# michel-aractingi/soloRL

Hardware: AMD Instinct MI355X
Metric: env-steps/s (whole node) Solo12 walk, 4096 envs/GPU (higher is better)
Workload: dtype f32

## Files before the change

### solorl_amd/csrc/dynamics.hpp

```cpp
#pragma once
#include <utility>

#include "../../include/solorl.h"
#include "../../include/solorl_model_data.h"
#include "spatial.hpp"

namespace solo {

constexpr int MAX_CONTACTS = 8;
constexpr int MAX_LIMITS = 4;
constexpr int LIM_SLOT_ROWS = 2;
constexpr int MAX_ROWS = LIM_SLOT_ROWS + 3 * MAX_CONTACTS;
SD int extra_limits(int nlt) { return nlt > LIM_SLOT_ROWS ? nlt - LIM_SLOT_ROWS : 0; }
SD int contact_cap(int nlt) { return MAX_CONTACTS - extra_limits(nlt); }
constexpr int ROW_CORE = 20;
constexpr int NPRIM = 24;
constexpr double LIMIT_WINDOW = 0.0;
constexpr double DISC_EPS2 = 1e-12;
constexpr double DISC_RIM = 0.1;

#if defined(SOLO_WAVE_TIMING) && !defined(SOLO_HOST_SHIM)
constexpr int SOLO_WT_WAVES = 65536, SOLO_WT_FIELDS = 30;
__device__ unsigned long long solo_wave_times[SOLO_WT_WAVES][SOLO_WT_FIELDS];
__shared__ unsigned long long solo_pt_acc[12];
#define SOLO_PT_DECL() long long pt_last_ = 0
#define SOLO_PT_BEGIN() do { __builtin_amdgcn_s_waitcnt(0); pt_last_ = clock64(); } while (0)
#define SOLO_PT(i) do { __builtin_amdgcn_s_waitcnt(0); if (threadIdx.x == 0) { const long long n_ = clock64(); solo_pt_acc[i] += (unsigned long long)(n_ - pt_last_); } pt_last_ = clock64(); } while (0)
#else
#define SOLO_PT_DECL() do {} while (0)
#define SOLO_PT_BEGIN() do {} while (0)
#define SOLO_PT(i) do {} while (0)
#endif

template <int N, typename F, int... I>
SD void static_for_impl(F&& f, std::integer_sequence<int, I...>) { (f(std::integral_constant<int, I>{}), ...); }
template <int N, typename F> SD void static_for(F&& f) { static_for_impl<N>(f, std::make_integer_sequence<int, N>{}); }

template <int ROBOT> struct Robot;
template <> struct Robot<0> {
  static constexpr int NJ = 2, NQ = 8, NL = 13;
  static constexpr bool SHOULDER = false;
  static constexpr const solorl_model_data& MD = SOLORL_MODEL_SOLO8;
};
template <> struct Robot<1> {
  static constexpr int NJ = 3, NQ = 12, NL = 17;
  static constexpr bool SHOULDER = true;
  static constexpr const solorl_model_data& MD = SOLORL_MODEL_SOLO12;
};

constexpr bool base_points_are_sign_patterns(const solorl_model_data& md) {
  const solorl_prim_data& a = md.prims[0]; const solorl_prim_data& b = md.prims[8];
  for (int p = 0; p < 12; p++) {
    const solorl_prim_data& q = md.prims[p];
    const bool plate = p >= 8;
    const double sx = ((plate ? (p - 8) >> 1 : p >> 2) & 1) ? -1.0 : 1.0, sy = ((plate ? (p - 8) : p >> 1) & 1) ? -1.0 : 1.0;
    const double cx = (plate ? b.center[0] : a.center[0]) * sx, cy = (plate ? b.center[1] : a.center[1]) * sy;
    const double cz = plate ? b.center[2] : ((p & 1) ? -a.center[2] : a.center[2]);
    if (q.link != 0 || q.axis != -1 || q.center[0] != cx || q.center[1] != cy || q.center[2] != cz || q.margin != a.margin || q.friction != a.friction) return false;
  }
  return true;
}

template <typename T> struct PhysParams {
  T dt, gravity, erp, slop, warm, damping, vmax, qlim, inv_dt;
  int iterations;
  T tm_hw, tm_mu;
  T resid_thr;
  T cerp;
  T cmargin;
  int mode;
  enum { M_PIPE = 1, M_URDF = 2, M_CONE = 4, M_TREADMILL = 8 };
  SD bool pgs_pipe() const { return mode & M_PIPE; }
  SD bool urdf_inertia() const { return mode & M_URDF; }
  SD bool cone() const { return mode & M_CONE; }
  SD bool tm_on() const { return mode & M_TREADMILL; }
  void set_mode(bool pipe, bool urdf, bool cone_, bool treadmill) {
    mode = (pipe ? M_PIPE : 0) | (urdf ? M_URDF : 0) | (cone_ ? M_CONE : 0) | (treadmill ? M_TREADMILL : 0);
  }
};
template <typename T> PhysParams<T> make_phys(const solorl_config& c) {
  PhysParams<T> p;
  p.dt = (T)c.sim_dt; p.gravity = (T)c.gravity; p.erp = (T)c.erp; p.slop = (T)c.linear_slop; p.warm = (T)c.warmstart;
  p.damping = (T)c.damping; p.vmax = (T)c.max_velocity; p.qlim = (T)c.joint_limit; p.inv_dt = (T)(1.0 / c.sim_dt);
  p.iterations = c.solver_iterations;
  p.tm_hw = (T)c.treadmill_half_width; p.tm_mu = (T)c.treadmill_friction;
  p.resid_thr = c.solver_residual_threshold > 0 ? (T)std::sqrt(c.solver_residual_threshold) : T(-1);
  p.cerp = (T)c.contact_erp; p.cmargin = (T)c.collision_margin;
  p.set_mode(true, c.use_urdf_inertia != 0, c.friction_model == SOLORL_FRICTION_CONE, c.use_treadmill != 0);
  return p;
}
SD int strip_feet_bits(int smask) {
  return (((smask >> 13) & 1) << 24) | (((smask >> 15) & 1) << 25) | (((smask >> 17) & 1) << 26) | (((smask >> 19) & 1) << 27);
}

template <typename T, int NQ> struct PhysState {
  V3<T> pos; T qx, qy, qz, qw; V3<T> v, w;
  T q[NQ], qd[NQ];
};

template <typename T> struct JointF { SV<T> S, U, c; T Dinv, u; };

#ifndef SOLO_HOST_SHIM
extern __shared__ __attribute__((aligned(16))) unsigned char solo_smem_sym[];
#if defined(SOLO_WAVE_TIMING)
constexpr unsigned SOLO_LDS_BASE = 96;
#else
constexpr unsigned SOLO_LDS_BASE = 0;
#endif
typedef __attribute__((address_space(3))) unsigned char solo_lds_byte;
#define solo_smem (((unsigned char*)reinterpret_cast<solo_lds_byte*>(SOLO_LDS_BASE + 4096u)) - 4096)
#endif
#ifdef SOLO_HOST_SHIM
template <typename T> constexpr int default_lanes() { return 1; }
#else
template <typename T> constexpr int default_lanes() { return sizeof(T) == 4 ? 64 : 32; }
#endif
template <typename T, int LN = default_lanes<T>()> struct RowLds {
  static constexpr int PER = 16 / sizeof(T);
  static constexpr int NCH = ROW_CORE / PER;
  static constexpr int LANES = LN;
  using Chunk = typename std::conditional<sizeof(T) == 4, float4, double2>::type;
  enum { A_MU = 0, A_LAM = 1, A_YOFF = 2, A_META = 3 };
  int lanes, lane;
#ifdef SOLO_HOST_SHIM
  unsigned char* base;
  SD unsigned char* smem() const { return base; }
#else
  SD unsigned char* smem() const { return solo_smem; }
#endif
  SD Chunk* core() const { return reinterpret_cast<Chunk*>(smem()) + lane; }
  SD T* aux() const { return reinterpret_cast<T*>(smem() + (size_t)MAX_ROWS * LANES * ROW_CORE * sizeof(T)) + lane; }
  SD T* y() const { return reinterpret_cast<T*>(smem() + (size_t)MAX_ROWS * LANES * (ROW_CORE + 4) * sizeof(T)) + lane; }
  SD T* hdr() const { return y() + 12 * LANES; }
  SD T& A(int r, int f) const { return aux()[(r * 4 + f) * LANES]; }

  SD void store_core(int r, const T (&v)[ROW_CORE]) const {
    Chunk* p = core() + r * (NCH * LANES);
#pragma unroll
    for (int c = 0; c < NCH; c++) {
      Chunk ch;
      if constexpr (sizeof(T) == 4) ch = make_float4(v[4 * c], v[4 * c + 1], v[4 * c + 2], v[4 * c + 3]);
      else ch = make_double2(v[2 * c], v[2 * c + 1]);
      p[c * LANES] = ch;
    }
  }
  SD void load_core(int r, T (&v)[ROW_CORE]) const {
    const Chunk* p = core() + r * (NCH * LANES);
#pragma unroll
    for (int c = 0; c < NCH; c++) {
      Chunk ch = p[c * LANES];
      if constexpr (sizeof(T) == 4) { v[4 * c] = ch.x; v[4 * c + 1] = ch.y; v[4 * c + 2] = ch.z; v[4 * c + 3] = ch.w; }
      else { v[2 * c] = ch.x; v[2 * c + 1] = ch.y; }
    }
  }
  static constexpr size_t bytes(int) {
    return (size_t)MAX_ROWS * LANES * (ROW_CORE + 4) * sizeof(T) + (size_t)(LANES == 4 ? 20 : 12) * LANES * sizeof(T);
  }
};

template <int OD = 0, typename T>
SD void link_terms(const M3<T>& R, V3<T> cw, T m, T ix, T iy, T iz, SV<T> v, T kd, RBI<T>& I, SV<T>& p, T ixy = T(0), T ixz = T(0),
                   T iyz = T(0)) {
  Sym3<T> Ic;
  Ic.xx = ix * R.c0.x * R.c0.x + iy * R.c1.x * R.c1.x + iz * R.c2.x * R.c2.x;
  Ic.xy = ix * R.c0.x * R.c0.y + iy * R.c1.x * R.c1.y + iz * R.c2.x * R.c2.y;
  Ic.xz = ix * R.c0.x * R.c0.z + iy * R.c1.x * R.c1.z + iz * R.c2.x * R.c2.z;
  Ic.yy = ix * R.c0.y * R.c0.y + iy * R.c1.y * R.c1.y + iz * R.c2.y * R.c2.y;
  Ic.yz = ix * R.c0.y * R.c0.z + iy * R.c1.y * R.c1.z + iz * R.c2.y * R.c2.z;
  Ic.zz = ix * R.c0.z * R.c0.z + iy * R.c1.z * R.c1.z + iz * R.c2.z * R.c2.z;
  auto add_od = [&](T w, const V3<T>& a, const V3<T>& b) {
    Ic.xx += T(2) * w * a.x * b.x; Ic.yy += T(2) * w * a.y * b.y; Ic.zz += T(2) * w * a.z * b.z;
    Ic.xy += w * (a.x * b.y + a.y * b.x); Ic.xz += w * (a.x * b.z + a.z * b.x); Ic.yz += w * (a.y * b.z + a.z * b.y);
  };
  if constexpr (OD & 1) add_od(ixy, R.c0, R.c1);
  if constexpr (OD & 2) add_od(ixz, R.c0, R.c2);
  if constexpr (OD & 4) add_od(iyz, R.c1, R.c2);
  V3<T> vc = v.l + cross(v.a, cw);
  V3<T> Icw = mul(Ic, v.a);
  T kl = kd + kd * sqrt_fast(dot(vc, vc));
  T ka = kd + kd * sqrt_fast(dot(v.a, v.a));
  V3<T> fc = (cross(v.a, vc) + vc * kl) * m;
  V3<T> nc = cross(v.a, Icw) + Icw * ka;
  p.a = nc + cross(cw, fc);
  p.l = fc;
  T cc = dot(cw, cw);
  I.m = m; I.h = cw * m;
  I.I.xx = Ic.xx + m * (cc - cw.x * cw.x); I.I.xy = Ic.xy - m * cw.x * cw.y; I.I.xz = Ic.xz - m * cw.x * cw.z;
  I.I.yy = Ic.yy + m * (cc - cw.y * cw.y); I.I.yz = Ic.yz - m * cw.y * cw.z;
// ... 1175 lines not shown
  T* hdr = lds.hdr();
  hdr[0] = T(nlt); hdr[LN] = T(nc);
}

template <typename T, int ROBOT, typename LDS, typename CH>
SD void phase_legrates_team(CH ch, const PhysParams<T> pp, const LDS lds, int t) {
  using RB = Robot<ROBOT>;
  using TRW = TeamRows<T, LDS>;
  constexpr int NJ = RB::NJ;
  T* bc = TRW::bc(lds.lane);
  if (t < RB::NQ) {
    SubCtx<T, ROBOT>& C = ch.get();
    const int L = t / NJ, k = t - L * NJ;
    const SV<T> a0{{bc[54], bc[55], bc[56]}, {bc[57], bc[58], bc[59]}};
    const T qdd = C.LR[L].qdd0[k] - dot(C.LR[L].G[k], a0);
    const T v = clampv(C.ps.qd[t] + pp.dt * qdd, pp.vmax);
    C.qds[t] = v;
    bc[42 + L * 3 + k] = v;
  } else if (NJ < 3 && t < 12) {
    if ((t - RB::NQ) < 4) bc[42 + (t - RB::NQ) * 3 + 2] = T(0);
  }
}

template <typename T, typename LDS> SD void team_counts(const LDS& lds, int& nlt, int& nc, int& ncmax, int& anylim) {
  const T* hdr = lds.hdr();
  nlt = (int)hdr[0]; nc = (int)hdr[LDS::LANES];
  int m = (nc + extra_limits(nlt)) | (nlt << 8);
#pragma unroll
  for (int o = 32; o >= 16; o >>= 1) { int v = __shfl_xor(m, o); m = ((v & 255) > (m & 255) ? (v & 255) : (m & 255)) | ((v | m) & ~255); }
  m = __builtin_amdgcn_readfirstlane(m);
  ncmax = m & 255; anylim = m >> 8;
}

template <typename T, int ROBOT, typename LDS>
SNI_SCALAR void phase_finish_team(const PhysParams<T> pp, const LDS lds, int t) {
  using TRW = TeamRows<T, LDS>;
  const int col = lds.lane;
  int nlt, nc, ncmax, anylim;
  team_counts<T, LDS>(lds, nlt, nc, ncmax, anylim);
  const int nrows = nlt + 3 * nc, rfric = nlt + nc;
  T* const lam = TRW::lam(col);
  const T* bc = TRW::bc(col);
  for (int pos = t; pos < TRW::TR; pos += 16)
    if (TRW::row_of(pos, nlt, nc) < 0) lam[pos * 4] = T(0);
  if (t >= nrows) return;
  Sym6<T> Lam;
#pragma unroll
  for (int i = 0; i < 6; i++)
#pragma unroll
    for (int j = 0; j < 6; j++) Lam.m[i][j] = bc[i * 6 + j];
  const SV<T> ub{{bc[36], bc[37], bc[38]}, {bc[39], bc[40], bc[41]}};
  const int r1 = t + 16;
  const bool two = r1 < nrows;
  T c0[ROW_CORE], c1[ROW_CORE];
  lds.load_core(t, c0);
  const int meta0 = (int)lds.A(t, LDS::A_META);
  const T mu0 = lds.A(t, LDS::A_MU);
  int meta1 = 0; T mu1 = T(1);
  if (two) { lds.load_core(r1, c1); meta1 = (int)lds.A(r1, LDS::A_META); mu1 = lds.A(r1, LDS::A_MU); }
  auto emit = [&](int r, const T (&c)[ROW_CORE], int meta, T mu) __attribute__((always_inline)) {
    const int leg = (meta >> 5) & 3;
    const T* ql = bc + 42 + leg * 3;
    SV<T> W; T rhs, dinv;
    finish_row(c, meta, Lam, ub, ql[0], ql[1], ql[2], pp, W, rhs, dinv);
    const bool fr = r >= rfric;
    const T sB = fr ? mu : T(1);
    const T isB = rcp_fast(sB);
    const T sJ = dinv * isB;
    T o[ROW_CORE];
#pragma unroll
    for (int e = 0; e < 9; e++) o[E_J(e)] = c[e] * sJ;
    o[E_B(0)] = W.a.x * sB; o[E_B(1)] = W.a.y * sB; o[E_B(2)] = W.a.z * sB; o[E_B(3)] = W.l.x * sB; o[E_B(4)] = W.l.y * sB; o[E_B(5)] = W.l.z * sB;
    o[E_B(6)] = c[15] * sB; o[E_B(7)] = c[16] * sB; o[E_B(8)] = c[17] * sB;
    o[E_RHS] = rhs * isB;
    o[E_LEG] = T(leg);
    lds.store_core(r, o);
    lds.A(r, LDS::A_LAM) = (fr && pp.cone()) ? rcp_fast(pp.resid_thr * sJ) : pp.resid_thr * sJ;
    lam[TRW::pos_of(r, nlt, nc) * 4] = c[13];
  };
  emit(t, c0, meta0, mu0);
  if (two) emit(r1, c1, meta1, mu1);
}

template <typename T> SD T half_swap(T x) {
  if constexpr (sizeof(T) == 4) return __int_as_float(__builtin_amdgcn_mov_dpp(__float_as_int(x), 0x140, 0xF, 0xF, true));
  else return __shfl_xor(x, 8, 16);
}

template <typename T> SD T team_red8(T x) {
  if constexpr (sizeof(T) == 4) {
    x += __int_as_float(__builtin_amdgcn_mov_dpp(__float_as_int(x), 0xB1, 0xF, 0xF, true));
    x += __int_as_float(__builtin_amdgcn_mov_dpp(__float_as_int(x), 0x4E, 0xF, 0xF, true));
    x += __int_as_float(__builtin_amdgcn_mov_dpp(__float_as_int(x), 0x141, 0xF, 0xF, true));
  } else {
    x += __shfl_xor(x, 1, 16); x += __shfl_xor(x, 2, 16); x += __shfl_xor(x, 4, 16);
  }
  return x;
}

#ifndef SOLO_SETUP_GROUP_F32
#define SOLO_SETUP_GROUP_F32 5
#endif
#ifndef SOLO_SETUP_GROUP_F64
#define SOLO_SETUP_GROUP_F64 1
#endif
#ifndef SOLO_K7_GATE_MIN_NFS
#define SOLO_K7_GATE_MIN_NFS 1
#endif
template <typename T, typename LDS, int LIM, int NNS, int NFS, bool EXIT, bool PIPE = true, bool CONE = false>
SNI void pgs_team_variant(int iterations_v, const LDS lds, int t) {
  using TRW = TeamRows<T, LDS>;
  const int itv = __builtin_amdgcn_readfirstlane(iterations_v);
  const int iterations = itv & 0xFFFF;
  const bool warm_on = (itv >> 30) & 1;
  constexpr int LN = LDS::LANES, n = LIM + NNS + NFS;
  constexpr int S_N0 = 1, S_F0 = 1 + MAX_CONTACTS / 2;
  static_assert(n >= 1, "empty sweeps are not instantiated");
  struct Ord { static constexpr int slot(int i) { return i < LIM ? 0 : (i < LIM + NNS ? S_N0 + (i - LIM) : S_F0 + (i - LIM - NNS)); } };
  const int col = lds.lane;
  const int h = t & 7, half = t >> 3;
  constexpr int SZ = (int)sizeof(T);
  constexpr int S_LAM = 4 * SZ;
  const int lam_own = (int)TRW::off_lam + col * SZ + half * S_LAM;
  const int nlt = (int)lds.hdr()[0], nc = (int)lds.hdr()[LN];
  const int eU = h;
  const int legU = h < 6 ? -1 : 0;
  const int eV = 6 + (h + 2) % 3, legV = (h + 2) / 3;
  const int eW = h < 2 ? 7 + h : 8, legW = h < 2 ? 3 : -2;
  constexpr unsigned ROWB = (unsigned)LDS::NCH * LN * 16u;
  auto eoff = [&](int e) -> unsigned { return (unsigned)(e / LDS::PER) * (LN * 16u) + (unsigned)(e % LDS::PER) * SZ + (unsigned)col * 16u; };
  using P2 = T __attribute__((ext_vector_type(2)));
  static_assert(LDS::PER % 2 == 0, "a (J', B~) pair lies inside one 16-byte chunk");
  const unsigned kU = eoff(E_J(eU)), kV = eoff(E_J(eV)), kW = eoff(E_J(eW));
  const unsigned kUB = eoff(E_B(eU)), kVB = eoff(E_B(eV)), kWB = eoff(E_B(eW));
  const unsigned kLEG = eoff(E_LEG), kRHS = eoff(E_RHS);
  auto rd = [&](unsigned rb, unsigned k) -> T { return *reinterpret_cast<const T*>(solo_smem + (rb + k)); };
  auto rd2 = [&](unsigned rb, unsigned k) -> P2 { return *reinterpret_cast<const P2*>(solo_smem + (rb + k)); };
  auto fm = [](auto a, auto b, auto c) { return __builtin_elementwise_fma(a, b, c); };
  T J0[n], J1[n], J2[n], B2[n], X2[n], rh[n], cp[n], lm[n], eo[n], ex[n];
  P2 B01[n], X01[n];
  T th[EXIT ? n : 1];
  T thx[(EXIT && CONE && NFS > 0) ? NFS : 1];
  T lmo[NNS > 0 ? NNS : 1];
  P2 a01 = {T(0), T(0)}; T a2 = T(0);
  int rown[n], roth[n];
  T lego[n], legx[n];
  T ju[n], bu[n], jv[n], bv[n], jw[n], bw[n], xu[n], xv[n], xw[n], rhs_[n];
  constexpr int SETUP_GROUP = sizeof(T) == 4 ? SOLO_SETUP_GROUP_F32 : SOLO_SETUP_GROUP_F64;
  static_for<(n + SETUP_GROUP - 1) / SETUP_GROUP>([&](auto gc) {
    constexpr int g0 = decltype(gc)::value * SETUP_GROUP, gn = (n - g0 < SETUP_GROUP ? n - g0 : SETUP_GROUP);
    static_for<gn>([&](auto jc) {
      constexpr int i = g0 + decltype(jc)::value;
      constexpr int k = Ord::slot(i);
      constexpr bool fr = i >= LIM + NNS;
      rown[i] = TRW::row_of(2 * k + half, nlt, nc);
      if constexpr (fr) roth[i] = rown[i] < 0 ? -1 : rown[i] + 1 - 2 * half;
      else roth[i] = TRW::row_of(2 * k + 1 - half, nlt, nc);
      const int ro = rown[i] < 0 ? 0 : rown[i], rx = roth[i] < 0 ? 0 : roth[i];
      const unsigned bo = __umul24((unsigned)ro, ROWB), bx = __umul24((unsigned)rx, ROWB);
      lego[i] = rd(bo, kLEG);
      if constexpr (!fr) legx[i] = rd(bx, kLEG); else legx[i] = T(0);
      { const P2 u = rd2(bo, kU), v = rd2(bo, kV), w = rd2(bo, kW);
        ju[i] = u.x; bu[i] = u.y; jv[i] = v.x; bv[i] = v.y; jw[i] = w.x; bw[i] = w.y; }
      xu[i] = rd(bx, kUB); xv[i] = rd(bx, kVB); xw[i] = rd(bx, kWB);
      rhs_[i] = rd(bo, kRHS);
      if constexpr (EXIT) th[i] = lds.A(ro, LDS::A_LAM);
      lm[i] = *reinterpret_cast<const T*>(solo_smem + lam_own + 2 * k * S_LAM);
    });
#ifndef SOLO_HOST_SHIM
    asm volatile("" ::: "memory");
    static_for<gn>([&](auto jc) {
      constexpr int i = g0 + decltype(jc)::value;
      asm volatile("" : "+v"(ju[i]), "+v"(bu[i]), "+v"(jv[i]), "+v"(bv[i]), "+v"(jw[i]), "+v"(bw[i]), "+v"(xu[i]), "+v"(xv[i]), "+v"(xw[i]),
                        "+v"(rhs_[i]), "+v"(lm[i]), "+v"(lego[i]));
      (void)legx;
      if constexpr (i < LIM + NNS) asm volatile("" : "+v"(legx[i]));
      (void)th;
      if constexpr (EXIT) asm volatile("" : "+v"(th[i]));
    });
#endif
    static_for<gn>([&](auto jc) {
      constexpr int i = g0 + decltype(jc)::value;
      constexpr bool fr = i >= LIM + NNS;
      const int r_own = rown[i], r_oth = roth[i];
      const int lo = r_own < 0 ? -3 : (int)lego[i], lx = fr ? lo : (r_oth < 0 ? -3 : (int)legx[i]);
      const bool uo = r_own >= 0 && (legU == -1 || legU == lo), vo = legV == lo, wo = legW == lo;
      const bool ux = fr ? uo : (r_oth >= 0 && (legU == -1 || legU == lx)), vx = fr ? vo : legV == lx, wx = fr ? wo : legW == lx;
      J0[i] = uo ? ju[i] : T(0); J1[i] = vo ? jv[i] : T(0); J2[i] = wo ? jw[i] : T(0);
      B01[i] = P2{uo ? bu[i] : T(0), vo ? bv[i] : T(0)}; B2[i] = wo ? bw[i] : T(0);
      X01[i] = P2{ux ? xu[i] : T(0), vx ? xv[i] : T(0)}; X2[i] = wx ? xw[i] : T(0);
      rh[i] = r_own >= 0 ? rhs_[i] * T(-0.125) : T(0);
      if constexpr (CONE && fr) {
        cp[i] = T(0);
        (void)thx;
        if constexpr (EXIT) { if (r_own < 0) th[i] = T(0); thx[i - LIM - NNS] = half_swap(th[i]); }
      } else {
        const T c = team_red8(J0[i] * X01[i].x + J1[i] * X01[i].y + J2[i] * X2[i]);
        cp[i] = half ? c : T(0);
      }
      if constexpr (i >= LIM && i < LIM + NNS) lmo[i - LIM] = T(0);
    });
    if (warm_on) {
      static_for<gn>([&](auto jc) {
        constexpr int i = g0 + decltype(jc)::value;
        const T lx_ = half_swap(lm[i]);
        if constexpr (i >= LIM && i < LIM + NNS) lmo[i - LIM] = lx_;
        a01 = fm(X01[i], P2{lx_, lx_}, fm(B01[i], P2{lm[i], lm[i]}, a01)); a2 = fm(X2[i], lx_, fm(B2[i], lm[i], a2));
      });
    }
  });
  static_for<n>([&](auto ic) {
    constexpr int i = decltype(ic)::value, p = (i + n - 1) % n;
    if constexpr (PIPE) {
      eo[i] = team_red8(J0[i] * B01[p].x + J1[i] * B01[p].y + J2[i] * B2[p]);
      ex[i] = team_red8(J0[i] * X01[p].x + J1[i] * X01[p].y + J2[i] * X2[p]);
    } else { eo[i] = T(0); ex[i] = T(0); (void)p; }
  });
  auto jdot = [&](int, T j0, T j1, T j2, T r8) -> T { return team_red8(fm(j0, a01.x, fm(j1, a01.y, fm(j2, a2, r8)))); };
  T dpre = jdot(0, J0[0], J1[0], J2[0], rh[0]);
  T delp = T(0), delxp = T(0);
  T* const hdr = lds.hdr();
#define SOLO_PGS_WRITE_BACK() do { \
    if (h == 0) { \
      static_for<n>([&](auto ic_) { \
        constexpr int i_ = decltype(ic_)::value; \
        *reinterpret_cast<T*>(solo_smem + lam_own + 2 * Ord::slot(i_) * S_LAM) = lm[i_]; \
      }); \
    } \
    if (half == 0) { \
      if (h < 6) hdr[(2 + h) * LN] = a01.x; else lds.y()[(h - 6) * LN] = a01.x; \
      lds.y()[(h + 2) * LN] = a01.y; \
      if (h < 2) lds.y()[(10 + h) * LN] = a2; \
    } } while (0)
  unsigned long long finm = 0; (void)finm;
  if constexpr (EXIT) finm = ~__builtin_amdgcn_ballot_w64(true);
#if defined(SOLO_WAVE_TIMING) && defined(SOLO_DEAD_STATS)
  unsigned long long fr_tot = 0, fr_dead = 0;
#endif
  int it_done = 0; (void)it_done;
  constexpr bool GATE = EXIT && CONE && NFS >= SOLO_K7_GATE_MIN_NFS && sizeof(T) == 4;
#pragma unroll 1
  for (int it = iterations; it > 0; it--) {
#if defined(SOLO_WAVE_TIMING) && defined(SOLO_SWEEP_STATS)
    it_done++;
#endif
    unsigned long long violm = 0; (void)violm;
    T vmax = T(0); (void)vmax;
    T dk[GATE ? NFS : 1], dkx[GATE ? NFS : 1]; (void)dk; (void)dkx;
    static_for<n>([&](auto ic) {
      constexpr int i = decltype(ic)::value, in = (i + 1) % n;
      constexpr bool fric = i >= LIM + NNS;
      T dnext = T(0), d = T(0), sv, del, delx, tx = T(0);
      (void)d; (void)tx;
#if defined(SOLO_WAVE_TIMING) && defined(SOLO_DEAD_STATS)
      constexpr bool SCHED = false, SCHEDN = false;
#else
      constexpr bool SCHED = PIPE && CONE && fric && sizeof(T) == 4;
      constexpr bool SCHEDN = PIPE && !fric && sizeof(T) == 4;
#endif
#define SOLO_SB() __builtin_amdgcn_sched_barrier(0)
#define SOLO_DPP_ADD(x_, ctrl_) ((x_) + __int_as_float(__builtin_amdgcn_mov_dpp(__float_as_int(x_), ctrl_, 0xF, 0xF, true)))
      if constexpr (SCHED) {
        constexpr int c = i - LIM - NNS;
        SOLO_SB();
        d = fm(ex[i], delxp, fm(eo[i], delp, dpre));
        const T sp = lm[i] - d;
        SOLO_SB();
        dnext = fm(J0[in], a01.x, fm(J1[in], a01.y, fm(J2[in], a2, rh[in])));
        SOLO_SB();
        const T spx = half_swap(sp);
        T s2 = fm(spx, spx, T(1e-30));
        SOLO_SB();
        dnext = SOLO_DPP_ADD(dnext, 0xB1);
        SOLO_SB();
        s2 = fm(sp, sp, s2);
        const T rs = __builtin_amdgcn_rsqf(s2);
        SOLO_SB();
        dnext = SOLO_DPP_ADD(dnext, 0x4E);
        SOLO_SB();
        const T hi = __int_as_float(__builtin_amdgcn_mov_dpp(__float_as_int(lm[LIM + (c >> 1)]), 0x150 + 8 * (c & 1), 0xF, 0xF, true));
        const T sc = __builtin_amdgcn_fmed3f(hi * rs, 0.0f, 1.0f);
        del = fm(sp, sc, -lm[i]);
        SOLO_SB();
        dnext = SOLO_DPP_ADD(dnext, 0x141);
        sv = sp * sc;
        if constexpr (EXIT && !GATE) tx = del * th[i];
        SOLO_SB();
        delx = half_swap(del);
        SOLO_SB();
      } else if constexpr (SCHEDN) {
        SOLO_SB();
        d = fm(ex[i], delxp, fm(eo[i], delp, dpre));
        T sp = lm[i] - d;
        const T dfirst = (sp > T(0) ? sp : T(0)) - lm[i];
        SOLO_SB();
        dnext = fm(J0[in], a01.x, fm(J1[in], a01.y, fm(J2[in], a2, rh[in])));
        SOLO_SB();
        sp = fm(-cp[i], half_swap(dfirst), sp);
        SOLO_SB();
        dnext = SOLO_DPP_ADD(dnext, 0xB1);
        SOLO_SB();
        sv = sp > T(0) ? sp : T(0);
        del = sv - lm[i];
        SOLO_SB();
        dnext = SOLO_DPP_ADD(dnext, 0x4E);
        a01 = fm(B01[i], P2{del, del}, a01);
        SOLO_SB();
        delx = half_swap(del);
        SOLO_SB();
        dnext = SOLO_DPP_ADD(dnext, 0x141);
        SOLO_SB();
      } else {
        if constexpr (PIPE) {
          dnext = jdot(in, J0[in], J1[in], J2[in], rh[in]);
          d = fm(ex[i], delxp, fm(eo[i], delp, dpre));
        } else d = jdot(i, J0[i], J1[i], J2[i], rh[i]);
        T hi = T(0);
        if constexpr (fric) {
          constexpr int c = i - LIM - NNS;
          if constexpr (sizeof(T) == 4) hi = __int_as_float(__builtin_amdgcn_mov_dpp(__float_as_int(lm[LIM + (c >> 1)]), 0x150 + 8 * (c & 1), 0xF, 0xF, true));
          else hi = (half == (c & 1)) ? lm[LIM + (c >> 1)] : lmo[c >> 1];
        }
        auto clampb = [&](T x) -> T {
// ... 201 lines not shown

template <typename T, int ROBOT, typename LDS, typename CH>
SNI_SCALAR void duo_integrate_joints(CH ch, const PhysParams<T> pp, const LDS lds, int t, bool valid) {
  using RB = Robot<ROBOT>;
  using TRW = TeamRows<T, LDS>;
  constexpr int NJ = RB::NJ, LN = LDS::LANES;
  if (!valid) return;
  SubCtx<T, ROBOT>& C = ch.get();
  const T dt = pp.dt;
  const int mask = C.mask;
  const int nlt = C.nlim_total;
  const T* hdr = lds.hdr();
  const SV<T> w{{hdr[2 * LN], hdr[3 * LN], hdr[4 * LN]}, {hdr[5 * LN], hdr[6 * LN], hdr[7 * LN]}};
  const int tj = t < RB::NQ ? t : 0;
  const int L = tj / NJ, k = tj - L * NJ;
  const T qds = C.qds[tj], yk = lds.y()[(L * 3 + k) * LN], qj = C.ps.q[tj];
  const SV<T> Gk = C.LR[L].G[k];
  const T* lam = TRW::lam(lds.lane);
  const int npos0 = TRW::NPOS0 + extra_limits(nlt);
  T lv[(NPRIM + 15) / 16];
#pragma unroll
  for (int i = 0; i < (NPRIM + 15) / 16; i++) {
    const int p = t + 16 * i;
    const int pp_ = p < NPRIM ? p : 0;
    lv[i] = lam[(npos0 + __builtin_popcount(mask & ((1 << pp_) - 1))) * 4];
    lv[i] = (p < NPRIM && ((mask >> pp_) & 1)) ? lv[i] : T(0);
  }
  const T nvj = clampv(qds + yk - dot(Gk, w), pp.vmax);
#pragma unroll
  for (int i = 0; i < (NPRIM + 15) / 16; i++) { const int p = t + 16 * i; if (p < NPRIM) C.lamp[p] = lv[i]; }
  if (t < RB::NQ) { C.ps.qd[t] = nvj; C.ps.q[t] = qj + dt * nvj; }
}

template <typename T, int ROBOT, typename LDS, typename CH>
SNI_SCALAR void duo_integrate_base(CH ch, const PhysParams<T> pp, const LDS lds, bool lead, bool r0) {
  constexpr int LN = LDS::LANES;
  if (!lead) return;
  SubCtx<T, ROBOT>& C = ch.get();
  const T dt = pp.dt;
  const T* hdr = lds.hdr();
  const SV<T> w{{hdr[2 * LN], hdr[3 * LN], hdr[4 * LN]}, {hdr[5 * LN], hdr[6 * LN], hdr[7 * LN]}};
  const SV<T> ub = C.ub;
  const V3<T> pos = C.ps.pos;
  const T x = C.ps.qx, yq = C.ps.qy, z = C.ps.qz, ww = C.ps.qw;
  const V3<T> nw = mk(clampv(ub.a.x + w.a.x, pp.vmax), clampv(ub.a.y + w.a.y, pp.vmax), clampv(ub.a.z + w.a.z, pp.vmax));
  const V3<T> nv = mk(clampv(ub.l.x + w.l.x, pp.vmax), clampv(ub.l.y + w.l.y, pp.vmax), clampv(ub.l.z + w.l.z, pp.vmax));
  C.ps.w = nw; C.ps.v = nv;
  C.ps.pos = fma3(nv, dt, pos);
  T wn2 = dot(nw, nw), wn = sqrt_fast(wn2), sc, s_, cw;
  sincos_t(T(0.5) * wn * dt, s_, cw);
  if (wn < T(1e-3)) sc = T(0.5) * dt - dt * dt * dt * T(1.0 / 48.0) * wn2; else sc = s_ * rcp_fast(wn);
  T ax = nw.x * sc, ay = nw.y * sc, az = nw.z * sc;
  T nx = cw * x + ax * ww + ay * z - az * yq;
  T ny = cw * yq - ax * z + ay * ww + az * x;
  T nz = cw * z + ax * yq - ay * x + az * ww;
  T nq = cw * ww - ax * x - ay * yq - az * z;
  T inv = rsqrt_fast(nx * nx + ny * ny + nz * nz + nq * nq);
  C.ps.qx = nx * inv; C.ps.qy = ny * inv; C.ps.qz = nz * inv; C.ps.qw = nq * inv;
  if (r0) C.R0 = quat_to_mat(C.ps.qx, C.ps.qy, C.ps.qz, C.ps.qw);
}

template <typename T, int ROBOT, typename LDS>
SD void substep_team_helper(const PhysParams<T> pp, const LDS& lds, int t, bool lead, bool valid, bool r0_next) {
  using CH = typename TeamCtx<T, ROBOT, LDS>::type;
  const CH ch{lds.lane};
  WG_SYNC();
  if (pp.urdf_inertia()) phase_front_team<T, ROBOT, LDS, CH, true, true>(ch, pp, lds, t, valid, lead);
  else phase_front_team<T, ROBOT, LDS, CH, false, true>(ch, pp, lds, t, valid, lead);
  WG_SYNC();
#if defined(SOLO_WAVE_TIMING)
  __builtin_amdgcn_s_waitcnt(0);
  const long long wt_h0_ = clock64();
#endif
  if (valid) team_sum_base<T, ROBOT, CH>(ch, t);
  if (lead) phase_base_lead<T, ROBOT, LDS, CH>(ch, pp, nullptr, 0u, lds);
  else if (!valid && t == 0) {
    lds.hdr()[0] = T(0); lds.hdr()[LDS::LANES] = T(0);
  }
#if defined(SOLO_WAVE_TIMING)
  __builtin_amdgcn_s_waitcnt(0);
  if (threadIdx.x == 64) solo_pt_acc[4] += (unsigned long long)(clock64() - wt_h0_);
#endif
  duo_helper_rates<T, ROBOT, LDS, CH>(ch, pp, lds, t, valid);
  duo_join_rows<T, ROBOT>();
#if defined(SOLO_WAVE_TIMING)
  __builtin_amdgcn_s_waitcnt(0);
  const long long wt_h1_ = clock64();
#endif
  duo_integrate_base<T, ROBOT, LDS, CH>(ch, pp, lds, lead, r0_next);
#if defined(SOLO_WAVE_TIMING)
  __builtin_amdgcn_s_waitcnt(0);
  if (threadIdx.x == 64) solo_pt_acc[11] += (unsigned long long)(clock64() - wt_h1_);
#endif
}

template <typename T, int ROBOT, typename LDS, bool DUO = false>
SD int substep_team(const PhysParams<T> pp, T* lam_prev, unsigned nstride, const LDS& lds, int t, bool lead, bool valid) {
  constexpr int LN = LDS::LANES;
  using TRW = TeamRows<T, LDS>;
  using CH = typename TeamCtx<T, ROBOT, LDS>::type;
  const CH ch{lds.lane};
  SOLO_PT_DECL();
  SOLO_PT_BEGIN();
  if (valid && t < Robot<ROBOT>::NQ) {
    SubCtx<T, ROBOT>& C = ch.get();
    T sn, cs;
    sincos_t(C.ps.q[t], sn, cs);
    C.sn[t] = sn; C.cs[t] = cs;
  }
  SOLO_PT(0);
  const bool ui = pp.urdf_inertia();
  if constexpr (DUO) WG_SYNC();
  else if (ui) phase_front_team<T, ROBOT, LDS, CH, true>(ch, pp, lds, t, valid, lead);
  else phase_front_team<T, ROBOT, LDS, CH, false>(ch, pp, lds, t, valid, lead);
  SOLO_PT(1);
#if SOLO_LEG_QUAD
  if constexpr (DUO) {
    if (ui) phase_leg_rt<T, ROBOT, LDS, CH, true, true>(ch, pp, lam_prev, nstride, lds, t >> 2, t & 3);
    else phase_leg_rt<T, ROBOT, LDS, CH, false, true>(ch, pp, lam_prev, nstride, lds, t >> 2, t & 3);
  } else if (valid) {
    if (ui) phase_leg_rt<T, ROBOT, LDS, CH, true>(ch, pp, lam_prev, nstride, lds, t >> 2, t & 3);
    else phase_leg_rt<T, ROBOT, LDS, CH, false>(ch, pp, lam_prev, nstride, lds, t >> 2, t & 3);
  }
#else
  static_assert(!DUO, "the helper wavefront's barrier B is in the quad leg phase");
  if (valid && t < 4) {
    if (ui) phase_leg_rt<T, ROBOT, LDS, CH, true>(ch, pp, lam_prev, nstride, lds, t, 0);
    else phase_leg_rt<T, ROBOT, LDS, CH, false>(ch, pp, lam_prev, nstride, lds, t, 0);
  }
#endif
  SOLO_PT(2);
  if constexpr (DUO) {
    duo_join_rows<T, ROBOT>();
    SOLO_PT(3);
  } else {
    if (valid) team_sum_base<T, ROBOT, CH>(ch, t);
    SOLO_PT(3);
    if (lead) phase_base_lead<T, ROBOT, LDS, CH>(ch, pp, lam_prev, nstride, lds);
    else if (!valid && t == 0) {
      lds.hdr()[0] = T(0); lds.hdr()[LN] = T(0);
    }
    SOLO_PT(4);
    if (valid) phase_legrates_team<T, ROBOT, LDS, CH>(ch, pp, lds, t);
    SOLO_PT(5);
  }
  phase_finish_team<T, ROBOT, LDS>(pp, lds, t);
  SOLO_PT(6);
  phase_pgs_team<T, ROBOT, LDS>(pp.iterations, pp.warm != T(0), pp.resid_thr >= T(0), pp.pgs_pipe(), pp.cone(), lds, t);
  SOLO_PT(7);
  if constexpr (DUO) {
    duo_join_rows<T, ROBOT>();
    SOLO_PT(10);
    duo_integrate_joints<T, ROBOT, LDS, CH>(ch, pp, lds, t, valid);
  } else phase_integrate_team<T, ROBOT, LDS, CH>(ch, pp, lam_prev, nstride, lds, t, valid, lead);
  SOLO_PT(8);
  return lead ? (ch.get().mask | strip_feet_bits(ch.get().smask)) : 0;
}
#endif

template <typename T, int ROBOT, typename LDS>
SD int substep(SubCtx<T, ROBOT>& C, const PhysParams<T> pp, T* lam_prev, unsigned nstride, const LDS& lds) {
  using CH = CtxPriv<T, ROBOT>;
  const CH ch{&C};
  if (pp.urdf_inertia()) {
    phase_detect<T, ROBOT, CH, true>(ch, pp);
    phase_leg<T, ROBOT, 0, LDS, CH, true>(ch, pp, lam_prev, nstride, lds);
    phase_leg<T, ROBOT, 1, LDS, CH, true>(ch, pp, lam_prev, nstride, lds);
    phase_leg<T, ROBOT, 2, LDS, CH, true>(ch, pp, lam_prev, nstride, lds);
    phase_leg<T, ROBOT, 3, LDS, CH, true>(ch, pp, lam_prev, nstride, lds);
  } else {
    phase_detect<T, ROBOT, CH, false>(ch, pp);
    phase_leg<T, ROBOT, 0, LDS, CH, false>(ch, pp, lam_prev, nstride, lds);
    phase_leg<T, ROBOT, 1, LDS, CH, false>(ch, pp, lam_prev, nstride, lds);
    phase_leg<T, ROBOT, 2, LDS, CH, false>(ch, pp, lam_prev, nstride, lds);
    phase_leg<T, ROBOT, 3, LDS, CH, false>(ch, pp, lam_prev, nstride, lds);
  }
  phase_base<T, ROBOT, LDS, CH>(ch, pp, lam_prev, nstride, lds);
  if (pp.cone()) phase_pgs<T, ROBOT, LDS, CH, true>(ch, pp.iterations, pp.resid_thr, lds);
  else phase_pgs<T, ROBOT, LDS, CH>(ch, pp.iterations, pp.resid_thr, lds);
  phase_integrate<T, ROBOT, LDS, CH>(ch, pp, lam_prev, nstride, lds);
  return C.mask | strip_feet_bits(C.smask);
}

}
```

### solorl_amd/csrc/solorl_hip.hip

```cpp
#include <hip/hip_runtime.h>

#include <cmath>
#include <cstddef>
#include <cstdio>
#include <cstdlib>
#include <cstring>
#include <utility>
#include <string>
#include <vector>

#include "../../include/solorl.h"
#include "dynamics.hpp"
#include "perturb.hpp"

using namespace solo;

#ifndef SOLO_TU_PART
#define SOLO_TU_PART -1
#endif
extern "C" __attribute__((visibility("hidden"))) int solorl_fail_(int code, const char* msg);

namespace {

#if SOLO_TU_PART == -1 || SOLO_TU_PART == 4
// ... 457 lines not shown
    }
}
SD void pol_act_store(const float (&c)[4], const float (&a)[4], unsigned yoff, int lane) {
#pragma unroll
  for (int e = 0; e < 4; e++) {
    float* y = reinterpret_cast<float*>(solo_smem + e * POL_ENV_BYTES + yoff);
    y[lane] = pol_tanh(c[e]); y[64 + lane] = pol_tanh(a[e]);
  }
}

template <int A>
SD void policy_tail_team(const PolicyTail& P, int O, int col, int t, idx_t env, bool valid) {
  float* const buf = reinterpret_cast<float*>(solo_smem + (unsigned)col * POL_ENV_BYTES);
  float* const h2 = buf + 224;
  const int lane = threadIdx.x & 63, O4 = O >> 2;
  static_assert(A < 15, "the critic head sits on lane 15");
  const bool head = t < A || t == 15;
  constexpr unsigned H1 = 96u * 4u, H2 = 224u * 4u;
  float c[4], a[4];
  PolBatch<11> w1a, w1b;
  PolBatch<8> w2a, w2b;
  nfloat4 whb[16];
  pol_load(w1a, P.cw0, P.aw0, O4, 0, lane);
  pol_load(w1b, P.cw0, P.aw0, O4, 11, lane);
#pragma unroll
  for (int e = 0; e < 4; e++) { c[e] = P.cb0[lane]; a[e] = P.ab0[lane]; }
  pol_fma(w1a, O4, 0, 0u, 0u, c, a);
  pol_load(w2a, P.cw1, P.aw1, 16, 0, lane);
  pol_fma(w1b, O4, 11, 0u, 0u, c, a);
  pol_act_store(c, a, H1, lane);
  pol_load(w2b, P.cw1, P.aw1, 16, 8, lane);
#pragma unroll
  for (int e = 0; e < 4; e++) { c[e] = P.cb1[lane]; a[e] = P.ab1[lane]; }
  TEAM_SYNC();
  pol_fma(w2a, 16, 0, H1, H1 + 256u, c, a);
  {
    gfloat4* wh = (gfloat4*)(t == 15 ? P.cw2 : P.mw + (size_t)(head ? t : 0) * 64);
#pragma unroll
    for (int k = 0; k < 16; k++) whb[k] = wh[k];
    asm volatile("" ::: "memory");
  }
  pol_fma(w2b, 16, 8, H1, H1 + 256u, c, a);
  pol_act_store(c, a, H2, lane);
  TEAM_SYNC();
  float out = 0.f;
  {
    asm volatile("" ::: "memory");
#pragma unroll
    for (int k = 0; k < 16; k++) POL_PIN4(whb[k]);
    const nfloat4* x = reinterpret_cast<const nfloat4*>(t == 15 ? h2 : h2 + 64);
    float o0 = t == 15 ? P.cb2[0] : P.mb[head ? t : 0], o1 = 0.f;
#pragma unroll
    for (int k = 0; k < 16; k += 2) { o0 = pol_dot4(whb[k], x[k], o0); o1 = pol_dot4(whb[k + 1], x[k + 1], o1); }
    out = head ? o0 + o1 : 0.f;
  }
  float lp = 0.f, act = out;
  if (t < A) {
    const float ls = P.logstd[t];
    const float nz = P.noise ? P.noise[(size_t)env * A + t] : 0.f;
    act = out + __expf(ls) * nz;
    lp = -0.5f * nz * nz - ls - POL_HALF_LOG_2PI;
  }
  lp = team_sum16(lp);
  if (valid) {
    if (t < A) P.action[(size_t)env * A + t] = act;
    if (t == 15) P.value[env] = out;
    if (t == 0) P.logp[env] = lp;
  }
}

template <typename T, int ROBOT, bool DUO = false>
SD void step_team(T* __restrict__ sf, int* __restrict__ si, const T* __restrict__ snf, const int* __restrict__ sni, int M,
                  const Layout& L, int N, const EnvParams& P, const PhysParams<T>& pp, const float* __restrict__ actions,
                  const Outputs& out, int mode) {
  using RB = Robot<ROBOT>;
  constexpr int NQ = RB::NQ, NPS = 13 + 2 * NQ;
  using LDS = RowLds<T, 4>;
  using CH = typename TeamCtx<T, ROBOT, LDS>::type;
  static_assert(sizeof(PhysState<T, NQ>) == NPS * sizeof(T), "PhysState is the HBM field order pos, quat, v, w, q, qd");
#ifdef SOLO_WAVE_TIMING
  long long wts_[11];
  for (int i_ = 0; i_ < 11; i_++) wts_[i_] = 0;
  const long long wr0_ = wall_clock64();
  if (threadIdx.x < 12) solo::solo_pt_acc[threadIdx.x] = 0;
  __syncthreads();
  wts_[0] = clock64();
#endif
  const unsigned wlane = DUO ? (threadIdx.x & 63u) : threadIdx.x;
  const int t = wlane & 15, col = wlane >> 4;
  const unsigned blk = (blockIdx.x & 7u) * (gridDim.x >> 3) + (blockIdx.x >> 3);
  idx_t e = (idx_t)blk * 4 + col;
  const bool valid = e < (idx_t)N;
  if (!valid) e = (idx_t)N - 1;
  const bool lead = valid && t == 0;
  LDS lds; lds.lanes = 4; lds.lane = col;
  if (P.lds_poison_on) {
    using TC = TeamCtx<T, ROBOT, LDS>;
    unsigned* w = reinterpret_cast<unsigned*>(solo_smem);
    for (unsigned k = wlane; k < TC::bytes / 4; k += 64) w[k] = P.lds_poison;
    __syncthreads();
  }
  const CH ch{col};
  SubCtx<T, ROBOT>& C = ch.get();
  T* const psv = reinterpret_cast<T*>(&C.ps);
  if constexpr (DUO) {
    if (blk * 4u >= (unsigned)N) return;
    if (__builtin_amdgcn_readfirstlane(threadIdx.x >> 6)) {
#pragma unroll 1
      for (int ss = 0; ss < P.frame_skip; ss++)
        substep_team_helper<T, ROBOT>(pp, lds, t, lead, valid, ss + 1 < P.frame_skip);
      duo_join_rows<T, ROBOT>();
      return;
    }
    if (!valid && t == 0) { C.mask = 0; C.nc = 0; C.nlim_total = 0; C.lsel = 0; C.smask = 0; }
  }
  idx_t env = 0;
  T a_t = T(0);
  if (valid) {
    env = P.linear_ids ? e : (idx_t)si[SX(I_ENVID, e, NI)];
    for (int f = t; f < NPS; f += 16) psv[f] = sf[SX(L.pos + f, e, L.NF)];
    if (t < NER) C.erec[t] = sf[SX(L.goal + t, e, L.NF)];
    if (t < 3) C.irec[t] = si[SX(t, e, NI)];
    for (int p = t; p < NPRIM; p += 16) C.lamp[p] = sf[SX(L.lam + p, e, L.NF)];
    if (t < NQ && mode == MODE_STEP) a_t = (T)actions[env * NQ + t];
  }
  static_assert(I_TIMESTEP == IR_TIMESTEP && I_MASK == IR_MASK && I_RNG == IR_RNG, "counter order");
  TEAM_SYNC();
  WT_STAMP(1);
  if (valid && t < NQ) {
    const T c = a_t < T(-1) ? T(-1) : (a_t > T(1) ? T(1) : a_t);
    T tq;
    if (P.control == SOLORL_CONTROL_TORQUE) tq = c * T(P.max_torque);
    else tq = clampv(T(P.kp) * (c * pp.qlim - C.ps.q[t]) - T(P.kd) * C.ps.qd[t], T(P.max_torque));
    C.tau_base[t] = mode == MODE_STEP ? tq : T(0);
    if (out.tau && mode == MODE_STEP) out.tau[env * NQ + t] = (float)tq;
  }
  const T asq = team_sum16(a_t * a_t);
  WT_STAMP(2);
  constexpr int HK = (DMAX + 15) / 16;
  T hk0[HK], hk1[HK];
#pragma unroll
  for (int k = 0; k < HK; k++) { hk0[k] = T(0); hk1[k] = T(0); }
  T csk[HK];
  if (L.H > 0) team_current_state<T, ROBOT, HK>(C, P.task, L.D, t, csk);
  TEAM_SYNC();
  if (lead) {
    C.erec[ER_XYPREV] = C.ps.pos.x; C.erec[ER_XYPREV + 1] = C.ps.pos.y;
    C.tmy = C.erec[ER_TMY];
    if constexpr (DUO) C.R0 = quat_to_mat(C.ps.qx, C.ps.qy, C.ps.qz, C.ps.qw);
  }
  if (valid && L.H > 0) {
#pragma unroll
    for (int k = 0; k < HK; k++) {
      const int d = t + 16 * k;
      if (d < L.D) {
        const T c = csk[k];
        for (int lv = L.H - 1; lv >= 2; lv--)
          sf[SX(L.hist + lv * HSTRIDE + d, e, L.NF)] = sf[SX(L.hist + (lv - 1) * HSTRIDE + d, e, L.NF)];
        if (L.H >= 2) { hk1[k] = sf[SX(L.hist + d, e, L.NF)]; sf[SX(L.hist + HSTRIDE + d, e, L.NF)] = hk1[k]; }
        sf[SX(L.hist + d, e, L.NF)] = c;
        hk0[k] = c;
      } else if (d < ((L.D + 3) & ~3)) {
        sf[SX(L.hist + d, e, L.NF)] = T(0);
        for (int lv = 1; lv < L.H; lv++) sf[SX(L.hist + lv * HSTRIDE + d, e, L.NF)] = T(0);
      }
    }
  }
// ... 46 lines not shown
      }
    }
    TEAM_SYNC();
    const T g0 = C.erec[ER_GOAL], g1 = C.erec[ER_GOAL + 1];
    if (P.task == SOLORL_TASK_POINTGOAL) {
#pragma unroll
      for (int kk = 0; kk < HK; kk++) {
        const int d = t + 16 * kk;
        if (d == L.D - 2 || d == L.D - 1) {
          const T gv = (d == L.D - 2 ? g0 : g1) * T(0.5);
          if (L.H >= 1) { hk0[kk] = gv; sf[SX(L.hist + d, e, L.NF)] = gv; }
          if (L.H >= 2) { hk1[kk] = gv; sf[SX(L.hist + HSTRIDE + d, e, L.NF)] = gv; }
          for (int lv = 2; lv < L.H; lv++) sf[SX(L.hist + lv * HSTRIDE + d, e, L.NF)] = gv;
        }
      }
    }
    if (t == 0) {
      C.irec[IR_TIMESTEP] = 0;
      C.erec[ER_GOALS] = T(0); C.erec[ER_EGOALS] = T(0);
#pragma unroll
      for (int q = 0; q < 5; q++) C.erec[ER_DR + q] = T(0);
      if (P.task == SOLORL_TASK_POINTGOAL) {
        const T dx = C.ps.pos.x - g0, dy = C.ps.pos.y - g1, px = C.erec[ER_XYPREV] - g0, py = C.erec[ER_XYPREV + 1] - g1;
        const T pot = sqrt(dx * dx + dy * dy);
        C.erec[ER_POT] = pot; C.erec[ER_PROG] = -(pot - sqrt(px * px + py * py));
      }
    }
  }
  WT_STAMP(7);
  const bool want_obs = mode == MODE_STEP;
  TEAM_SYNC();
  T cso[HK];
  if (want_obs) team_current_state<T, ROBOT, HK>(C, P.task, L.D, t, cso);
  WT_STAMP(8);
  bool with_policy = false;
  if constexpr (sizeof(T) == 4) with_policy = want_obs && out.pol.value != nullptr;
  if (valid) {
    if (want_obs) {
      float* o = out.obs + env * (idx_t)(L.D * (1 + L.H));
      float* ol = reinterpret_cast<float*>(solo_smem + (unsigned)col * POL_ENV_BYTES);
#pragma unroll
      for (int k = 0; k < HK; k++) {
        const int d = t + 16 * k;
        if (d < L.D) {
          const T c = cso[k];
          o[d] = (float)c;
          if (L.H >= 1) o[L.D + d] = (float)(c - hk0[k]);
          if (L.H >= 2) o[2 * L.D + d] = (float)(c - hk1[k]);
          for (int lv = 2; lv < L.H; lv++) {
            T hv;
            if (done) {
              hv = snf[SX(L.hist + lv * HSTRIDE + d, (idx_t)C.irec[IR_SNAP], L.NF)];
              if (P.task == SOLORL_TASK_POINTGOAL && d >= L.D - 2) hv = C.erec[ER_GOAL + (d - (L.D - 2))] * T(0.5);
            } else hv = sf[SX(L.hist + lv * HSTRIDE + d, e, L.NF)];
            o[(lv + 1) * L.D + d] = (float)(c - hv);
          }
          if (with_policy) {
            ol[d] = (float)c;
            if (L.H >= 1) ol[L.D + d] = (float)(c - hk0[k]);
          }
        }
      }
    }
    for (int f = t; f < ((NPS + 3) & ~3); f += 16) sf[SX(L.pos + f, e, L.NF)] = f < NPS ? psv[f] : T(0);
    sf[SX(L.goal + t, e, L.NF)] = t < NER ? C.erec[t] : T(0);
    if (t < 3) si[SX(t, e, NI)] = C.irec[t];
  }
  if constexpr (sizeof(T) == 4) {
    if (with_policy) {
      TEAM_SYNC();
      policy_tail_team<NQ>(out.pol, L.D * (1 + L.H), col, t, env, valid);
    }
  }
  WT_STAMP(9);
#ifdef SOLO_WAVE_TIMING
  __builtin_amdgcn_s_waitcnt(0);
  if (threadIdx.x == 0 && blockIdx.x < solo::SOLO_WT_WAVES) {
    wts_[10] = clock64();
    unsigned long long* w_ = solo::solo_wave_times[blockIdx.x];
    w_[0] = (unsigned long long)(wts_[3] - wts_[0]); w_[1] = (unsigned long long)(wts_[4] - wts_[3]); w_[2] = (unsigned long long)(wts_[10] - wts_[4]);
    w_[3] = (unsigned long long)(wall_clock64() - wr0_);
    for (int i_ = 0; i_ < 10; i_++) w_[6 + i_] = (unsigned long long)(wts_[i_ + 1] > wts_[i_] && wts_[i_] ? wts_[i_ + 1] - wts_[i_] : 0);
    for (int i_ = 0; i_ < 10; i_++) w_[16 + i_] = solo::solo_pt_acc[i_];
    for (int i_ = 10; i_ < 12; i_++) w_[18 + i_] = solo::solo_pt_acc[i_];
  }
#endif
}

template <typename T, int ROBOT>
__global__ void __launch_bounds__(64)
step_kernel(T* __restrict__ sf, int* __restrict__ si, const T* __restrict__ snf, const int* __restrict__ sni, int M,
            Layout L, int N, EnvParams P, PhysParams<T> pp, const float* __restrict__ actions, Outputs out, int mode) {
  step_body<T, ROBOT>(sf, si, snf, sni, M, L, N, P, pp, actions, out, mode);
}

#ifndef SOLO_WAVES_PER_SIMD
#define SOLO_WAVES_PER_SIMD 2
#endif
template <typename T, int ROBOT>
__global__ void __launch_bounds__(64, sizeof(T) == 8 ? 1 : SOLO_WAVES_PER_SIMD)
step_kernel_team(T* __restrict__ sf, int* __restrict__ si, const T* __restrict__ snf, const int* __restrict__ sni, int M,
                 Layout L, int N, EnvParams P, PhysParams<T> pp, const float* __restrict__ actions, Outputs out, int mode) {
  step_team<T, ROBOT>(sf, si, snf, sni, M, L, N, P, pp, actions, out, mode);
}

template <typename T, int ROBOT>
__global__ void __launch_bounds__(128, SOLO_WAVES_PER_SIMD)
duo_kernel_team(T* __restrict__ sf, int* __restrict__ si, const T* __restrict__ snf, const int* __restrict__ sni, int M,
                Layout L, int N, EnvParams P, PhysParams<T> pp, const float* __restrict__ actions, Outputs out, int mode) {
  static_assert(sizeof(T) == 4, "the helper wavefront is an fp32 kernel");
  step_team<T, ROBOT, true>(sf, si, snf, sni, M, L, N, P, pp, actions, out, mode);
}

template <typename T> struct RolloutArgs {
  T* sf; int* si; const T* snf; const int* sni; int M;
  Layout L; int N; EnvParams P; PhysParams<T> pp;
  const float* actions; Outputs out;
  int mode;
  int K, pol_last;
};
template <typename T> SD T* row_adv(T* p, size_t n) { return p ? p + n : p; }
template <typename T, int ROBOT>
__global__ void __launch_bounds__(64, sizeof(T) == 8 ? 1 : SOLO_WAVES_PER_SIMD)
rollout_kernel_team(const RolloutArgs<T> args) {
  using RA = RolloutArgs<T>;
  typedef const __attribute__((address_space(4))) char* kptr;
  constexpr size_t A = Robot<ROBOT>::NQ;
  const int K = args.K;
#pragma unroll 1
  for (int k = 0; k < K; k++) {
    kptr ap = (kptr)__builtin_amdgcn_kernarg_segment_ptr();
    asm volatile("" : "+s"(ap));
    const RA& a = *(const RA*)ap;
    const size_t r = (size_t)k * (size_t)a.N, O = (size_t)(a.L.D * (1 + a.L.H));
    Outputs o = a.out;
    o.obs += r * O; o.rew += r; o.done += r;
    o.timeout = row_adv(o.timeout, r); o.success = row_adv(o.success, r); o.nan_reset = row_adv(o.nan_reset, r);
    o.ep_len = row_adv(o.ep_len, r); o.ep_rew = row_adv(o.ep_rew, r); o.goals = row_adv(o.goals, r);
    o.dr0 = row_adv(o.dr0, r); o.dr1 = row_adv(o.dr1, r); o.dr2 = row_adv(o.dr2, r); o.dr3 = row_adv(o.dr3, r); o.dr4 = row_adv(o.dr4, r);
    o.tau = row_adv(o.tau, r * A);
    if (o.pol.value) {
      if (k + 1 < K || a.pol_last) {
        const size_t r1 = r + (size_t)a.N;
        o.pol.value += r1; o.pol.logp += r1; o.pol.action += r1 * A; o.pol.noise = row_adv(o.pol.noise, r1 * A);
      } else o.pol.value = nullptr;
    }
    step_team<T, ROBOT>(a.sf, a.si, a.snf, a.sni, a.M, a.L, a.N, a.P, a.pp, a.actions + r * A, o, a.mode);
    TEAM_SYNC();
  }
}

template <typename T, int ROBOT, bool MASKED>
__global__ void reset_kernel(T* sf, int* si, const T* snf, const int* sni, int M, Layout L, int N, EnvParams P, float* obs,
                             const unsigned char* mask) {
  const idx_t e = (idx_t)blockIdx.x * blockDim.x + threadIdx.x;
  if (e >= (idx_t)N) return;
  if constexpr (MASKED) { if (!mask[si[SX(I_ENVID, e, NI)]]) return; }
  Env<T, Robot<ROBOT>::NQ> E;
  load_env(E, sf, si, L, (idx_t)N, e);
  const idx_t env = (idx_t)si[SX(I_ENVID, e, NI)];
  reset_from_snapshot<T, ROBOT>(E, sf, L, (idx_t)N, e, env, snf, sni, M, P);
  if (obs) write_obs<T, ROBOT>(E, sf, L, (idx_t)N, e, env, P.task, obs);
  store_env(E, sf, si, L, (idx_t)N, e);
  si[SX(I_NEEDRESET, e, NI)] = 0;
}

template <typename T, int ROBOT>
// ... 1031 lines not shown
```

Before: 28.86 million.

## Split row finishing between main and helper waves in duo mode

In the two-wave (DUO) team step, the constraint-row finish phase is split. The main wave finishes rows 0-15 and the helper wave finishes rows 16+ right after its rate work, with an extra join barrier before PGS. Previously the main wave ran phase_finish_team over all rows alone. This moves serial per-row work onto the otherwise idle helper, at the cost of an additional cross-wave synchronisation. Timing instrumentation slots are also extended.

Result: faster. 29.22 million (median of 6 runs) (+1.2%).

```diff
diff --git a/solorl_amd/csrc/dynamics.hpp b/solorl_amd/csrc/dynamics.hpp
--- a/solorl_amd/csrc/dynamics.hpp
+++ b/solorl_amd/csrc/dynamics.hpp
@@ -20,9 +20,9 @@
 constexpr double DISC_RIM = 0.1;
 
 #if defined(SOLO_WAVE_TIMING) && !defined(SOLO_HOST_SHIM)
-constexpr int SOLO_WT_WAVES = 65536, SOLO_WT_FIELDS = 30;
+constexpr int SOLO_WT_WAVES = 65536, SOLO_WT_FIELDS = 32;
 __device__ unsigned long long solo_wave_times[SOLO_WT_WAVES][SOLO_WT_FIELDS];
-__shared__ unsigned long long solo_pt_acc[12];
+__shared__ unsigned long long solo_pt_acc[16];
 #define SOLO_PT_DECL() long long pt_last_ = 0
 #define SOLO_PT_BEGIN() do { __builtin_amdgcn_s_waitcnt(0); pt_last_ = clock64(); } while (0)
 #define SOLO_PT(i) do { __builtin_amdgcn_s_waitcnt(0); if (threadIdx.x == 0) { const long long n_ = clock64(); solo_pt_acc[i] += (unsigned long long)(n_ - pt_last_); } pt_last_ = clock64(); } while (0)
@@ -103,7 +103,7 @@
 #ifndef SOLO_HOST_SHIM
 extern __shared__ __attribute__((aligned(16))) unsigned char solo_smem_sym[];
 #if defined(SOLO_WAVE_TIMING)
-constexpr unsigned SOLO_LDS_BASE = 96;
+constexpr unsigned SOLO_LDS_BASE = 128;
 #else
 constexpr unsigned SOLO_LDS_BASE = 0;
 #endif
@@ -1445,6 +1445,51 @@
   if (two) emit(r1, c1, meta1, mu1);
 }
 
+template <typename T, int ROBOT, typename LDS, bool SECOND>
+SNI_SCALAR void duo_finish_rows(const PhysParams<T> pp, const LDS lds, int t) {
+  using TRW = TeamRows<T, LDS>;
+  const int col = lds.lane;
+  const T* hdr = lds.hdr();
+  const int nlt = (int)hdr[0], nc = (int)hdr[LDS::LANES];
+  const int nrows = nlt + 3 * nc, rfric = nlt + nc;
+  T* const lam = TRW::lam(col);
+  const T* bc = TRW::bc(col);
+  const int r = SECOND ? t + 16 : t;
+  if (r < TRW::TR && TRW::row_of(r, nlt, nc) < 0) lam[r * 4] = T(0);
+  if (r >= nrows) return;
+  Sym6<T> Lam;
+#pragma unroll
+  for (int i = 0; i < 6; i++)
+#pragma unroll
+    for (int j = 0; j < 6; j++) Lam.m[i][j] = bc[i * 6 + j];
+  const SV<T> ub{{bc[36], bc[37], bc[38]}, {bc[39], bc[40], bc[41]}};
+  T c[ROW_CORE];
+  lds.load_core(r, c);
+  const int meta = (int)lds.A(r, LDS::A_META);
+  const T mu = lds.A(r, LDS::A_MU);
+  auto emit = [&](int r, const T (&c)[ROW_CORE], int meta, T mu) __attribute__((always_inline)) {
+    const int leg = (meta >> 5) & 3;
+    const T* ql = bc + 42 + leg * 3;
+    SV<T> W; T rhs, dinv;
+    finish_row(c, meta, Lam, ub, ql[0], ql[1], ql[2], pp, W, rhs, dinv);
+    const bool fr = r >= rfric;
+    const T sB = fr ? mu : T(1);
+    const T isB = rcp_fast(sB);
+    const T sJ = dinv * isB;
+    T o[ROW_CORE];
+#pragma unroll
+    for (int e = 0; e < 9; e++) o[E_J(e)] = c[e] * sJ;
+    o[E_B(0)] = W.a.x * sB; o[E_B(1)] = W.a.y * sB; o[E_B(2)] = W.a.z * sB; o[E_B(3)] = W.l.x * sB; o[E_B(4)] = W.l.y * sB; o[E_B(5)] = W.l.z * sB;
+    o[E_B(6)] = c[15] * sB; o[E_B(7)] = c[16] * sB; o[E_B(8)] = c[17] * sB;
+    o[E_RHS] = rhs * isB;
+    o[E_LEG] = T(leg);
+    lds.store_core(r, o);
+    lds.A(r, LDS::A_LAM) = (fr && pp.cone()) ? rcp_fast(pp.resid_thr * sJ) : pp.resid_thr * sJ;
+    lam[TRW::pos_of(r, nlt, nc) * 4] = c[13];
+  };
+  emit(r, c, meta, mu);
+}
+
 template <typename T> SD T half_swap(T x) {
   if constexpr (sizeof(T) == 4) return __int_as_float(__builtin_amdgcn_mov_dpp(__float_as_int(x), 0x140, 0xF, 0xF, true));
   else return __shfl_xor(x, 8, 16);
@@ -1473,6 +1518,9 @@
 template <typename T, typename LDS, int LIM, int NNS, int NFS, bool EXIT, bool PIPE = true, bool CONE = false>
 SNI void pgs_team_variant(int iterations_v, const LDS lds, int t) {
   using TRW = TeamRows<T, LDS>;
+#if defined(SOLO_WAVE_TIMING)
+  const long long wt_su0_ = clock64();
+#endif
   const int itv = __builtin_amdgcn_readfirstlane(iterations_v);
   const int iterations = itv & 0xFFFF;
   const bool warm_on = (itv >> 30) & 1;
@@ -1602,6 +1650,10 @@
 #endif
   int it_done = 0; (void)it_done;
   constexpr bool GATE = EXIT && CONE && NFS >= SOLO_K7_GATE_MIN_NFS && sizeof(T) == 4;
+#if defined(SOLO_WAVE_TIMING)
+  __builtin_amdgcn_s_waitcnt(0);
+  if (threadIdx.x == 0) solo_pt_acc[13] += (unsigned long long)(clock64() - wt_su0_);
+#endif
 #pragma unroll 1
   for (int it = iterations; it > 0; it--) {
 #if defined(SOLO_WAVE_TIMING) && defined(SOLO_SWEEP_STATS)
@@ -1969,6 +2021,8 @@
   if (threadIdx.x == 64) solo_pt_acc[4] += (unsigned long long)(clock64() - wt_h0_);
 #endif
   duo_helper_rates<T, ROBOT, LDS, CH>(ch, pp, lds, t, valid);
+  duo_finish_rows<T, ROBOT, LDS, true>(pp, lds, t);
+  duo_join_rows<T, ROBOT>();
   duo_join_rows<T, ROBOT>();
 #if defined(SOLO_WAVE_TIMING)
   __builtin_amdgcn_s_waitcnt(0);
@@ -2031,8 +2085,15 @@
     if (valid) phase_legrates_team<T, ROBOT, LDS, CH>(ch, pp, lds, t);
     SOLO_PT(5);
   }
-  phase_finish_team<T, ROBOT, LDS>(pp, lds, t);
-  SOLO_PT(6);
+  if constexpr (DUO) {
+    duo_finish_rows<T, ROBOT, LDS, false>(pp, lds, t);
+    SOLO_PT(6);
+    duo_join_rows<T, ROBOT>();
+    SOLO_PT(12);
+  } else {
+    phase_finish_team<T, ROBOT, LDS>(pp, lds, t);
+    SOLO_PT(6);
+  }
   phase_pgs_team<T, ROBOT, LDS>(pp.iterations, pp.warm != T(0), pp.resid_thr >= T(0), pp.pgs_pipe(), pp.cone(), lds, t);
   SOLO_PT(7);
   if constexpr (DUO) {
diff --git a/solorl_amd/csrc/solorl_hip.hip b/solorl_amd/csrc/solorl_hip.hip
--- a/solorl_amd/csrc/solorl_hip.hip
+++ b/solorl_amd/csrc/solorl_hip.hip
@@ -563,7 +563,7 @@
   long long wts_[11];
   for (int i_ = 0; i_ < 11; i_++) wts_[i_] = 0;
   const long long wr0_ = wall_clock64();
-  if (threadIdx.x < 12) solo::solo_pt_acc[threadIdx.x] = 0;
+  if (threadIdx.x < 16) solo::solo_pt_acc[threadIdx.x] = 0;
   __syncthreads();
   wts_[0] = clock64();
 #endif
@@ -776,7 +776,7 @@
     w_[3] = (unsigned long long)(wall_clock64() - wr0_);
     for (int i_ = 0; i_ < 10; i_++) w_[6 + i_] = (unsigned long long)(wts_[i_ + 1] > wts_[i_] && wts_[i_] ? wts_[i_ + 1] - wts_[i_] : 0);
     for (int i_ = 0; i_ < 10; i_++) w_[16 + i_] = solo::solo_pt_acc[i_];
-    for (int i_ = 10; i_ < 12; i_++) w_[18 + i_] = solo::solo_pt_acc[i_];
+    for (int i_ = 10; i_ < 14; i_++) w_[18 + i_] = solo::solo_pt_acc[i_];
   }
 #endif
 }
```
